# yuw444/fastF

Measured on AMD Instinct MI355X. Metric: BAM records/sec -> deduped UMI matrix; achieved HBM GB/s vs roofline, higher is better.
Workload: dtype u64

## Files before the change

fastf_amd/csrc/umi_engine.hip:

```cpp
#include "umi_kernels.hpp"

#include <algorithm>
#include <cstdarg>
#include <cstdio>
#include <cstdlib>
#include <cstring>
#include <mutex>
#include <new>
#include <stdexcept>
#include <chrono>
#include <string>
#include <thread>
#include <vector>

extern "C" {
#include "fastf_amd.h"
#include "host_io.h"
#include "mt_jump.h"
}

using namespace fastf;

static std::mutex g_err_mu;
static char g_err[512] = "";
// ... 191 lines not shown
    std::vector<uint8_t> h_unonnull;
    u64 total_records = 0, hits_so_far = 0, keys_so_far = 0;
    u64 c_sampled = 0, c_valid = 0;
    bool finished = false; int sorted_in_tmp = 0; u64 n_sorted = 0;
    u32 skip_bits = 0;
    bool fully_sorted = false;
    DevBuf d_cellidx, d_tilecnt, d_tilebase, d_binbase, d_cnt;
    DevBuf d_halfhits;
    DevBuf d_segkeys;
    DevBuf d_segcount, d_segprefix, d_tileseg;
    u32 giant_parity = 0;
    u32 seg_n = 0; u64 seg_stride = 0;
    DevBuf d_rgn_phys, d_rgn_hist, d_rgn_blk;
    u32 rgn_hist_n = 0, rgn_hist_shift = 0;
    bool stream_mode = false, store_regions = false;
    u64 slots_used = 0, slot_cap = 0; u32 rgn_n = 0, rgn_cap = 0;
    DevBuf d_scanblk;
    DevBuf d_rg_feature, d_rg_cell, d_rg_count, d_rg_ukeys, d_spanrows, d_spanbase, d_giant;
    u32 rg_n = 0; bool rg_umi = false;
    bool wide = false, long_umi = false; u32 group_bits = 0;
    u32 sub_bits = 0, row_split = 0;
    bool finish_queued = false;
    DevBuf d_vals, d_vtmp;
    bool timing = false;
    hipEvent_t t_ev[2] = {nullptr, nullptr};
    double t_scatter_ms = 0; u64 t_scatter_n = 0;
    double t_k1_ms = 0; u64 t_k1_n = 0;
    double t_k1b_ms = 0; u64 t_k1b_n = 0;
    double t_k3_ms = 0; u64 t_k3_n = 0;
    double t_count_ms = 0; u64 t_count_n = 0;
// ... 192 lines not shown
        for (u32 w = 0; w < words; ++w) { rank[w] = (unsigned short)acc; acc += (u32)__builtin_popcount(bitmap[w]); }
    }
    if (e->img_genes.ensure(bytes)) return 1;
    if (copy_h2d(e->img_genes.p, img.data(), bytes)) return 1;
    e->lds_genes.image = (const u32*)e->img_genes.p; e->lds_genes.words = words; e->lds_genes.n_perm = (u32)best_n;
    e->lds_genes.family = (u32)best; e->lds_genes.vmin = vmin; e->lds_genes.range = range; e->lds_genes.bytes = (u32)bytes; e->lds_genes.direct = direct ? 1u : 0u;
    {
        const void* fns[] = {(const void*)filter_pack_kernel<true, false>, (const void*)filter_pack_kernel<true, true>,
                             (const void*)filter_pack_stream_kernel<false, false, false>, (const void*)filter_pack_stream_kernel<false, false, true>,
                             (const void*)filter_pack_stream_kernel<false, true, false>, (const void*)filter_pack_stream_kernel<false, true, true>,
                             (const void*)filter_pack_stream_kernel<true, false, false>, (const void*)filter_pack_stream_kernel<true, false, true>,
                             (const void*)filter_pack_stream_kernel<true, true, false>, (const void*)filter_pack_stream_kernel<true, true, true>,
                             (const void*)filter_pack_stream_kernel<false, false, false, true>, (const void*)filter_pack_stream_kernel<false, false, true, true>,
                             (const void*)filter_pack_stream_kernel<false, true, false, true>, (const void*)filter_pack_stream_kernel<false, true, true, true>,
                             (const void*)filter_pack_stream_kernel<true, false, false, true>, (const void*)filter_pack_stream_kernel<true, false, true, true>,
                             (const void*)filter_pack_stream_kernel<true, true, false, true>, (const void*)filter_pack_stream_kernel<true, true, true, true>};
        for (const void* f : fns)
            if (hipFuncSetAttribute(f, hipFuncAttributeMaxDynamicSharedMemorySize, (int)bytes) != hipSuccess) return 0;
    }
    const size_t per_block = bytes + 1024;
    e->genes_blocks_per_cu = (u32)std::max<size_t>(1, std::min<size_t>(3, (160 * 1024) / per_block));
    e->use_lds_genes = true;
    return 0;
}

extern "C" int fastf_engine_create(const fastf_engine_config_t* cfg, fastf_engine_t** out) FASTF_TRY {
    if (!cfg || !out) return set_err("null argument");
    *out = nullptr;
    const char* pf_ = getenv("FASTF_PROFILE");
    const bool lap_on = pf_ && pf_[0] == '2';
    const auto t_0 = std::chrono::steady_clock::now();
    auto lap = [&](const char* what) { if (lap_on) fprintf(stderr, "[engine create] %s at %.1f ms\n", what, std::chrono::duration<double, std::milli>(std::chrono::steady_clock::now() - t_0).count()); };
    int ndev = 0;
    hipError_t he = hipGetDeviceCount(&ndev);
    lap("device count");
    if (he != hipSuccess || ndev == 0)
        return set_err("no HIP device available (%s): the engine has no CPU fallback", hipGetErrorString(he));
// ... 76 lines not shown
        }
        lap("tables built and uploaded");
        if ((rc = e->d_small.ensure(SM_WORDS * sizeof(u64)))) break;
        if (hipHostMalloc((void**)&e->h_small, SM_WORDS * sizeof(u64), hipHostMallocDefault) != hipSuccess) {
            rc = set_err("hipHostMalloc failed"); break;
        }
        if (hipMemset(e->d_small.p, 0, SM_WORDS * sizeof(u64)) != hipSuccess) { rc = set_err("memset failed"); break; }
        lap("counters allocated and cleared");
        if (set_scatter_lds_limit()) {
            rc = set_err("cannot raise dynamic LDS limit to %zu bytes", scatter_smem_bytes()); break;
        }
        lap("kernel attributes (code object loaded)");
        e->batch_cap = cfg->batch_records ? cfg->batch_records : (4ull << 20);
        e->key_cap = cfg->key_capacity;
        e->stream_mode = e->use_lds_genes && !e->wide && e->n_shards == 1 && !getenv("FASTF_NO_STREAM_K1B") && !getenv("FASTF_PUSH_TILE_FORM");
    } while (0);
    if (rc) { fastf_engine_destroy(e); return 1; }
    *out = e;
    return 0;
} FASTF_CATCH_INT

extern "C" void fastf_engine_destroy(fastf_engine_t* e) FASTF_TRY {
    if (!e) return;
    if (e->multi) { multi_destroy(e); delete e; return; }
    (void)hipSetDevice(e->device);
    (void)hipDeviceSynchronize();
    for (int i = 0; i < 2; ++i) {
        fastf_engine::Slot& sl = e->slot[i];
        if (sl.h_stage) (void)hipHostFree(sl.h_stage);
        if (sl.h_draws) (void)hipHostFree(sl.h_draws);
// ... 130 lines not shown
    constexpr u32 CHUNK = 16u * 1024u;
    const u32 n_blk = (T + CHUNK - 1) / CHUNK;
    if (n_blk <= 1 || n_blk > 64 || e->d_scanblk.ensure(2 * 64 * sizeof(u64))) {
        hipLaunchKernelGGL(scan_tiles_kernel<16>, dim3(1), dim3(1024), 0, s, in, out, T, total_out, running, base_out, (u64*)nullptr);
        return;
    }
    u64* const blk = (u64*)e->d_scanblk.p + 64 * slot;
    hipLaunchKernelGGL(scan_tiles_kernel<16>, dim3(n_blk), dim3(1024), 0, s, in, out, T, (u64*)nullptr, (u64*)nullptr, (u64*)nullptr, blk);
    hipLaunchKernelGGL(scan_fix_kernel<16>, dim3(n_blk), dim3(1024), 0, s, out, T, (const u64*)blk, n_blk, total_out, running, base_out);
}

static int launch_probe_cells(fastf_engine* e, const u64* cb, u64 n, u64* d_total_out, hipStream_t s,
                              u64* d_running = nullptr, u64* d_base_out = nullptr, void* blk = nullptr) {
    if (reserve_workspace(e, blk ? 0 : n, 0, n)) return 1;
    const u32 tiles = (u32)((n + K1_TILE - 1) / K1_TILE);
    const CellOut cout = blk ? CellOut{blk, blk_run_bytes(e->cell16)} : CellOut{e->d_cellidx.p, 0u};
    t_begin(e, s);
    if (e->use_lds_cells) {
        const u32 grid = std::min<u32>(e->cells_blocks_per_cu * g_cu_count, (tiles + 1) / 2);
        if (e->cells_blocks_per_cu >= 2)
            hipLaunchKernelGGL(probe_cells_lds_kernel<true>, dim3(grid), dim3(1024), e->lds_cells.bytes, s, cb, n, e->lds_cells,
                               cout, e->cell16, (u32*)e->d_tilecnt.p, (u32*)e->d_halfhits.p, tiles);
        else
            hipLaunchKernelGGL(probe_cells_lds_kernel<false>, dim3(grid), dim3(1024), e->lds_cells.bytes, s, cb, n, e->lds_cells,
                               cout, e->cell16, (u32*)e->d_tilecnt.p, (u32*)e->d_halfhits.p, tiles);
    } else if (e->cell_filter.bits) {
        const u32 grid = std::min<u32>(tiles, 4 * g_cu_count);
        hipLaunchKernelGGL(probe_cells_filtered_kernel, dim3(grid), dim3(K1_THREADS), (e->cell_filter.mask + 1u) / 8u, s, cb, n,
                           e->cells, e->cell_filter, cout, e->cell16, (u32*)e->d_tilecnt.p, (u32*)e->d_halfhits.p, tiles);
    } else {
        hipLaunchKernelGGL(probe_cells_kernel<0>, dim3(tiles), dim3(K1_THREADS), 0, s, cb, n, e->cells,
// ... 13 lines not shown
    if (e->multi) return set_err("fastf_dev_count_hits: device-level calls take a single-device engine");
    HIP_OK(hipSetDevice(e->device));
    hipStream_t s = (hipStream_t)stream;
    if (n == 0) { HIP_OK(hipMemsetAsync(d_hits_out, 0, sizeof(u64), s)); return 0; }
    return launch_probe_cells(e, (const u64*)d_cb_key, n, (u64*)d_hits_out, s);
} FASTF_CATCH_INT

static bool stream_k1b_possible(const fastf_engine* e) {
    return e->use_lds_genes && e->n_shards <= (u32)MAX_SHARDS && !getenv("FASTF_NO_STREAM_K1B");
}

extern "C" int fastf_dev_block_bytes(const fastf_engine_t* e, uint64_t n, uint64_t* bytes) FASTF_TRY {
    if (!e || !bytes) return set_err("null argument");
    *bytes = 0;
    if (e->multi || e->wide || !stream_k1b_possible(e)) return 0;
    *bytes = ((n + BLK_RECS - 1) / BLK_RECS) * (u64)blk_run_bytes(e->cell16);
    return 0;
} FASTF_CATCH_INT

extern "C" int fastf_dev_block_records(fastf_engine_t* e, const uint64_t* d_gx_key, const uint32_t* d_umi, const uint32_t* d_meta,
                                       uint64_t n, void* d_blocked, void* stream) FASTF_TRY {
    if (!e || !d_blocked) return set_err("null argument");
    if (e->multi) return set_err("fastf_dev_block_records: device-level calls take a single-device engine");
    HIP_OK(hipSetDevice(e->device));
    if (n == 0) return 0;
    const u64 units = (n + BLK_RECS - 1) / BLK_RECS;
    hipLaunchKernelGGL(block_records_kernel, dim3((u32)std::min<u64>((units + 3) / 4, 16ull * g_cu_count)), dim3(256), 0, (hipStream_t)stream,
                       (const u64*)d_gx_key, d_umi, d_meta, (u64)n, (unsigned char*)d_blocked, blk_run_bytes(e->cell16));
    HIP_OK(hipGetLastError());
    dbg_sync((hipStream_t)stream, "block_records");
    return 0;
} FASTF_CATCH_INT

extern "C" int fastf_dev_count_hits_blocked(fastf_engine_t* e, const uint64_t* d_cb_key, uint64_t n, void* d_blocked,
                                            uint64_t* d_hits_out, void* stream) FASTF_TRY {
    if (!e || !d_blocked) return set_err("null argument");
    if (e->multi) return set_err("fastf_dev_count_hits_blocked: device-level calls take a single-device engine");
    HIP_OK(hipSetDevice(e->device));
    hipStream_t s = (hipStream_t)stream;
    if (n == 0) { HIP_OK(hipMemsetAsync(d_hits_out, 0, sizeof(u64), s)); return 0; }
    return launch_probe_cells(e, (const u64*)d_cb_key, n, (u64*)d_hits_out, s, nullptr, nullptr, d_blocked);
} FASTF_CATCH_INT

// ... 149 lines not shown
            if (e->d_segkeys.ensure((size_t)n_rgn * region * sizeof(u64))) return 1;
            p.keys = (u64*)e->d_segkeys.p;
        } else if ((u64)n_rgn * region > stride) return set_err("segmented key output needs %llu slots, the buffer has %llu (fastf_dev_probe_capacity)",
                                                                (unsigned long long)((u64)n_rgn * region), (unsigned long long)stride);
        if (app) {
            if (e->rgn_cap < rgn0 + n_rgn) return set_err("internal error: region tables too small");
        } else {
            if (e->rgn_n) return set_err("device-level K1 on an engine that holds pushed chunks: fastf_engine_reset first");
            if (grow_regions(e, n_rgn)) return 1;
        }
        if (e->d_segprefix.ensure(((size_t)n_rgn + 1) * sizeof(u64))) return 1;
        StreamParams sp{(const u32*)e->d_halfhits.p, region, (u64*)e->d_segcount.p + rgn0,
                        stream_shards ? nullptr : (u32*)e->d_rgn_hist.p + (size_t)rgn0 * RADIX, (u64*)e->d_rgn_phys.p + rgn0,
                        app ? app->slot0 : 0ull, e->skip_bits};
        const int variant = (e->genes_blocks_per_cu >= 2 ? 0 : 4) | (e->cell16 ? 2 : 0) | (e->lds_genes.direct ? 1 : 0);
#define FPS(R, C, D) do { if (blk) hipLaunchKernelGGL((filter_pack_stream_kernel<R, C, D, true>), dim3(grid), dim3(R ? K1S_THREADS_ROOMY : K1S_THREADS), e->lds_genes.bytes, s, p, sp); \
                          else hipLaunchKernelGGL((filter_pack_stream_kernel<R, C, D, false>), dim3(grid), dim3(R ? K1S_THREADS_ROOMY : K1S_THREADS), e->lds_genes.bytes, s, p, sp); } while (0)
        switch (variant) {
        case 0: FPS(false, false, false); break; case 1: FPS(false, false, true); break;
        case 2: FPS(false, true, false); break;  case 3: FPS(false, true, true); break;
        case 4: FPS(true, false, false); break;  case 5: FPS(true, false, true); break;
        case 6: FPS(true, true, false); break;   default: FPS(true, true, true); break;
        }
#undef FPS
        if (stream_shards) {
            hipLaunchKernelGGL(shard_partition_kernel, dim3(n_rgn), dim3(SP_THREADS), 0, s, (const u64*)e->d_segkeys.p, (const u64*)e->d_segcount.p,
                               region, e->L.cell_shift, e->n_shards, keys, stride, key_counts, counters + 3);
        } else if (app) {
            hipLaunchKernelGGL(seg_scan_kernel, dim3(1), dim3(1024), 0, s, (const u64*)e->d_segcount.p + rgn0, n_rgn, (u64*)e->d_segprefix.p, key_counts, true);
        } else {
            hipLaunchKernelGGL(seg_scan_kernel, dim3(1), dim3(1024), 0, s, (const u64*)e->d_segcount.p, n_rgn, (u64*)e->d_segprefix.p, key_counts, false);
// ... 333 lines not shown
           "block_records_kernel,tile_count_kernel,row_scan_kernel,scatter_kernel,reduce_windows_kernel,reduce_hashed_kernel,span_scan_kernel,"
           "giant_groups_kernel,rows_gather_kernel";
} FASTF_CATCH_ZERO

static const char* err_bits_text(u64 bits) {
    static thread_local char buf[256];
    snprintf(buf, sizeof buf, "device error bits 0x%llx:%s%s%s%s%s", (unsigned long long)bits,
             (bits & 1) ? " (unknown bit 0);" : "",
             (bits & ERR_DRAWS_SHORT) ? " draw stream shorter than CB hits;" : "",
             (bits & ERR_UMI_TOOLONG) ? " UMI longer than umi_max_bases (raise it: up to 32, with fastf_batch_t.umi_ext from 17 on);" : "",
             (bits & ERR_KEYS_FULL) ? " key store full;" : "",
             (bits & ERR_RUN_TOO_LONG) ? " unsorted run longer than the group-only path handles: sort fully (drop FASTF_SORT_SKIP_LOW);" : "");
    return buf;
}

static size_t stage_bytes(u64 cap) { return (size_t)cap * (8 + 8 + 4 + 4 + 4) + 8192; }


static int slot_alloc(fastf_engine* e, fastf_engine::Slot& sl, bool need_host_stage) {
    if (!sl.h_small) HIP_OK(hipHostMalloc((void**)&sl.h_small, SM_WORDS * sizeof(u64), hipHostMallocDefault));
    if (sl.d_stage.ensure(stage_bytes(e->batch_cap))) return 1;
    if (need_host_stage && !sl.h_stage) HIP_OK(hipHostMalloc(&sl.h_stage, stage_bytes(e->batch_cap), hipHostMallocDefault));
    return 0;
}

static int retire_slot(fastf_engine* e, fastf_engine::Slot& sl) {
    if (!sl.busy) return 0;
    HIP_OK(hipEventSynchronize(sl.ev_done));
    sl.busy = false;
    e->inflight_records -= sl.n;
    const u64* c = sl.h_small + SM_COUNTERS;
    if (!sl.external) e->mt_hits += c[0] - e->hits_so_far;
    e->hits_so_far = c[0];
    e->c_sampled = c[1]; e->c_valid = c[2];
    e->keys_so_far = sl.h_small[SM_KEYCOUNT];
    if (c[3]) return set_err("%s", err_bits_text(c[3]));
// ... 137 lines not shown
        const bool par = n >= (1u << 18);
        if (par) {
            t_gx = std::thread([=] { memcpy(hs + o_gx, s_gx, n * 8); });
            t_um = std::thread([=] { memcpy(hs + o_umi, s_umi, n * 4); memcpy(hs + o_meta, s_meta, n * 4); });
        } else {
            memcpy(hs + o_gx, s_gx, n * 8); memcpy(hs + o_umi, s_umi, n * 4); memcpy(hs + o_meta, s_meta, n * 4);
        }
        memcpy(hs, s_cb, n * 8);
        if (s_ext) { memcpy(hs + o_ext, s_ext, n * 4); s_ext = hs + o_ext; }
        if (par) { t_gx.join(); t_um.join(); }
        s_cb = hs; s_gx = hs + o_gx; s_umi = hs + o_umi; s_meta = hs + o_meta;
    }
    hipStream_t sc = e->s_copy, sk = e->s_compute;
    HIP_OK(hipMemcpyAsync(ds, s_cb, n * 8, hipMemcpyDefault, sc));
    char* const blk = ds + cap * 8;
    if (e->stream_mode) {
        const u32 run = blk_run_bytes(e->cell16);
        const u64 full = n / BLK_RECS, tail = n % BLK_RECS;
        if (full) {
            HIP_OK(hipMemcpy2DAsync(blk + BLK_GX, run, s_gx, BLK_RECS * 8, BLK_RECS * 8, full, hipMemcpyDefault, sc));
            HIP_OK(hipMemcpy2DAsync(blk + BLK_UMI, run, s_umi, BLK_RECS * 4, BLK_RECS * 4, full, hipMemcpyDefault, sc));
            HIP_OK(hipMemcpy2DAsync(blk + BLK_META, run, s_meta, BLK_RECS * 4, BLK_RECS * 4, full, hipMemcpyDefault, sc));
        }
        if (tail) {
            char* const last = blk + full * run;
            HIP_OK(hipMemcpyAsync(last + BLK_GX, (const char*)s_gx + full * BLK_RECS * 8, tail * 8, hipMemcpyDefault, sc));
            HIP_OK(hipMemcpyAsync(last + BLK_UMI, (const char*)s_umi + full * BLK_RECS * 4, tail * 4, hipMemcpyDefault, sc));
            HIP_OK(hipMemcpyAsync(last + BLK_META, (const char*)s_meta + full * BLK_RECS * 4, tail * 4, hipMemcpyDefault, sc));
        }
    } else {
    HIP_OK(hipMemcpyAsync(ds + o_gx, s_gx, n * 8, hipMemcpyDefault, sc));
// ... 514 lines not shown
```

fastf_amd/csrc/umi_kernels.hpp:

```cpp
#pragma once
#if !defined(FASTF_EXPERIMENT)
#  if defined(FASTF_X_ANY)
#    error "FASTF_X_* knobs need -DFASTF_EXPERIMENT (experiment builds only: tools/build_variant.sh)"
#  endif
#endif
#ifndef FASTF_K1_IPT
#define FASTF_K1_IPT 8
#endif
#ifndef FASTF_K1_THREADS
#define FASTF_K1_THREADS 512
#endif
#include <hip/hip_runtime.h>
#include <stdint.h>
#include <type_traits>

namespace fastf {

typedef unsigned long long u64;
typedef unsigned int u32;

constexpr int WAVE = 64;

constexpr u64 ERR_DRAWS_SHORT  = 2;
constexpr u64 ERR_UMI_TOOLONG  = 4;
// ... 290 lines not shown
        k |= (1ULL << (L.umi_bits + L.len_bits)) | ((u64)(umi >> (32 - L.umi_bits)) << L.len_bits) | len;
    }
    return k;
}

__device__ __forceinline__ u64 make_key_flat(const KeyLayout L, u32 cell, u32 feat, u32 umi, u32 meta) {
    const u32 nn = (meta / META_UMI_NONNULL) & 1u, len = (meta & META_LEN_MASK) >> META_LEN_SHIFT;
    const u64 low = ((u64)nn << (L.umi_bits + L.len_bits)) | ((u64)(umi >> (32 - L.umi_bits)) << L.len_bits) | len;
    return ((u64)cell << L.cell_shift) | ((u64)feat << L.feat_shift) | (low & (0ull - (u64)nn));
}
__device__ __forceinline__ bool umi_overflows_flat(const KeyLayout L, u32 umi, u32 meta) {
    const u32 tail = L.umi_bits < 32 ? (1u << (32 - L.umi_bits)) - 1u : 0u;
    const u32 len = (meta & META_LEN_MASK) >> META_LEN_SHIFT;
    return ((meta & META_UMI_TOOLONG) != 0) | (((meta & META_UMI_NONNULL) != 0) & ((len > L.umi_max_bytes) | ((umi & tail) != 0)));
}

__device__ __forceinline__ u64 make_val64(const KeyLayout L, u64 umi, u32 meta) {
    if (!(meta & META_UMI_NONNULL)) return 0;
    const u32 len = (meta & META_LEN_MASK) >> META_LEN_SHIFT;
    return (1ULL << (L.umi_bits + L.len_bits)) | ((umi >> (64 - L.umi_bits)) << L.len_bits) | len;
}
constexpr u32 WIDE_SUB_BITS = 17, WIDE_SUB_VAL_BITS = 51, WIDE_SUB_LEN_BITS = 4;
__device__ __forceinline__ u64 make_val_sub(u64 umi, u32 meta) {
    if (!(meta & META_UMI_NONNULL)) return 0;
    const u32 len = (meta & META_LEN_MASK) >> META_LEN_SHIFT;
    return (1ULL << WIDE_SUB_VAL_BITS) | (((umi << WIDE_SUB_LEN_BITS) | len) & ((1ULL << WIDE_SUB_VAL_BITS) - 1));
}
__device__ __forceinline__ u32 wide_sub_of(u32 umi_first_word, u32 meta) {
    static_assert(WIDE_SUB_VAL_BITS - WIDE_SUB_LEN_BITS + WIDE_SUB_BITS == 64, "the sub-group and the value's bases make up the 64 bits of bases");
    return (meta & META_UMI_NONNULL) ? umi_first_word >> (32 - WIDE_SUB_BITS) : 0u;
// ... 109 lines not shown
    u64 off = 0, total = 0;
    for (u32 i = 0; i < n_blk; ++i) { const u64 v = blk_tot[i]; if (i < blockIdx.x) off += v; total += v; }
    if (blockIdx.x == 0 && threadIdx.x == 0) {
        if (total_out) *total_out = total;
        if (running) { const u64 r = *running; *base_out = r; *running = r + total; }
    }
    if (blockIdx.x == 0 || off == 0) return;
    const u32 t_first = blockIdx.x * PER * 1024u;
    for (u32 k = threadIdx.x; k < PER * 1024u && t_first + k < T; k += 1024) out[t_first + k] += off;
}

constexpr int K1_THREADS = FASTF_K1_THREADS, K1_IPT = FASTF_K1_IPT, K1_TILE = K1_THREADS * K1_IPT, K1_WAVES = K1_THREADS / WAVE;
static_assert(K1_THREADS == 512 && K1_IPT == 8, "K1a layout: 8 waves x 8 items x 64 lanes per tile");

constexpr u32 BLK_RECS = 256, BLK_GX = 0, BLK_UMI = 2048, BLK_META = 3072, BLK_CELL = 4096;
__host__ __device__ __forceinline__ u32 blk_run_bytes(bool c16) { return BLK_CELL + (c16 ? 2u : 4u) * BLK_RECS; }
struct CellOut { void* p; u32 run; };
__device__ __forceinline__ void put_cell(const CellOut o, bool c16, u64 idx, u32 v) {
    unsigned char* at = reinterpret_cast<unsigned char*>(o.p);
    u64 i = idx;
    if (o.run) { at += (idx / BLK_RECS) * o.run + BLK_CELL; i = idx % BLK_RECS; }
    if (c16) reinterpret_cast<unsigned short*>(at)[i] = (unsigned short)v; else reinterpret_cast<u32*>(at)[i] = v;
}
__device__ __forceinline__ u32 get_cell(const void* __restrict__ in, bool c16, u64 idx) {
    return c16 ? (u32)reinterpret_cast<const unsigned short*>(in)[idx] : reinterpret_cast<const u32*>(in)[idx];
}

__device__ __forceinline__ u32 get_cell_once(const void* __restrict__ in, bool c16, u64 idx) {
    return c16 ? (u32)ld_once<FASTF_NT_K1B != 0>(reinterpret_cast<const unsigned short*>(in) + idx)
               : ld_once<FASTF_NT_K1B != 0>(reinterpret_cast<const u32*>(in) + idx);
}

__device__ __forceinline__ u32 shard_of(u32 cell, u32 n_shards) {
    return (u32)((mix64((u64)cell) >> 32) % n_shards);
}

// ... 133 lines not shown
        }
        u32 hits = 0, hits_lo = 0;
#pragma unroll
        for (int j = 0; j < K1_IPT; ++j) {
            const bool fam = (u32)(key[j] >> 49) == c.family && (key[j] & 0xFFFFu) == 0;
            const u32 h = cell_mix((u32)(key[j] >> 16), c.seed);
            const u32 lo = h & lo_mask;
            const u32 e = s_slot[((h >> (32u - S)) + s_disp[lo & c.bucket_mask]) & smask];
            const u32 v = (fam && (e >> S) == lo) ? (e & smask) : 0u;
            cell[j] = v;
            hits += (u32)__popcll(__ballot(v != 0));
            if (j == K1_IPT / 2 - 1) hits_lo = hits;
        }
        if (whole && cell_dst.run) {
            static_assert(K1_IPT * WAVE == 2 * (int)BLK_RECS && PAIRS == 4, "a K1a chunk is two blocked units");
            unsigned char* const u0 = reinterpret_cast<unsigned char*>(cell_out) + (base / BLK_RECS) * cell_dst.run + BLK_CELL;
#pragma unroll
            for (int j = 0; j < PAIRS; ++j) {
                unsigned char* const ub = u0 + (j >> 1) * cell_dst.run;
                const u32 rec = 2u * ((u32)(j & 1) * WAVE + (u32)lane);
                if (c16) *reinterpret_cast<u32*>(ub + 2u * rec) = cell[2 * j] | (cell[2 * j + 1] << 16);
                else *reinterpret_cast<uint2*>(ub + 4u * rec) = make_uint2(cell[2 * j], cell[2 * j + 1]);
            }
        } else if (whole) {
            if (c16) {
#pragma unroll
                for (int j = 0; j < PAIRS; ++j)
                    *reinterpret_cast<u32*>(reinterpret_cast<unsigned short*>(cell_out) + base + 2ull * (j * WAVE + lane)) = cell[2 * j] | (cell[2 * j + 1] << 16);
            } else {
#pragma unroll
                for (int j = 0; j < PAIRS; ++j)
// ... 272 lines not shown
    u64* seg_count;
    u32* rgn_hist;
    u64* rgn_phys;
    u64 slot0;
    u32 hist_shift;
};

__device__ __forceinline__ u32 row16_sum_lane15(u32 x) {
    x += (u32)__builtin_amdgcn_update_dpp(0, (int)x, 0x111, 0xF, 0xF, true);
    x += (u32)__builtin_amdgcn_update_dpp(0, (int)x, 0x112, 0xF, 0xF, true);
    x += (u32)__builtin_amdgcn_update_dpp(0, (int)x, 0x114, 0xF, 0xF, true);
    x += (u32)__builtin_amdgcn_update_dpp(0, (int)x, 0x118, 0xF, 0xF, true);
    return (u32)__builtin_amdgcn_readlane((int)x, 15);
}

template <bool ROOMY, bool C16, bool DIRECT, bool BLOCKED = false>
__global__ __launch_bounds__(ROOMY ? K1S_THREADS_ROOMY : K1S_THREADS, ROOMY ? 4 : 2 * K1S_THREADS / (4 * WAVE)) void filter_pack_stream_kernel(const PackParams p, const StreamParams sp) {
    constexpr int THREADS = ROOMY ? K1S_THREADS_ROOMY : K1S_THREADS, WAVES = THREADS / WAVE;
    __shared__ u64 s_tot[3];
    __shared__ u32 s_cursor[K1S_SUB], s_err;
    __shared__ u32 s_hist[K1S_SUB * K1S_BINS];
    extern __shared__ __attribute__((aligned(16))) unsigned char smem[];
    const int tid = threadIdx.x, lane = lane_id();
    const int w = __builtin_amdgcn_readfirstlane(tid >> 6);
    const u32* s_bitmap = reinterpret_cast<const u32*>(smem);
    const unsigned short* s_rank = reinterpret_cast<const unsigned short*>(smem + (size_t)p.genes.words * 4);
    const unsigned short* s_perm = s_rank + ((p.genes.words + 1u) & ~1u);
    const unsigned short* s_direct = reinterpret_cast<const unsigned short*>(smem);
    {
        const uint4* src = reinterpret_cast<const uint4*>(p.genes.image);
        uint4* dst = reinterpret_cast<uint4*>(smem);
        for (u32 i = tid; i < (p.genes.bytes + 15u) / 16u; i += THREADS) dst[i] = src[i];
    }
    if (tid < 3) s_tot[tid] = 0;
    if (tid < K1S_SUB) s_cursor[tid] = 0;
    if (tid == 0) s_err = 0;
    for (int i = tid; i < K1S_SUB * K1S_BINS; i += THREADS) s_hist[i] = 0;
    __syncthreads();

    constexpr bool NT = FASTF_NT_K1B != 0;
    u64* const region0 = p.keys + (u64)blockIdx.x * K1S_SUB * sp.region_stride;
    const bool hs_hi = sp.hist_shift >= 32u;
    const u64 draw_off = p.draw_base ? *p.draw_base : 0;
    u32 w_hit = 0, w_samp = 0, w_valid = 0, errs = 0;
    const u32 n_units = p.n_tiles * (u32)(K1_TILE / K1S_UNIT), ustep = gridDim.x * (u32)WAVES;
    const u32 n_live = (u32)((p.n + K1S_UNIT - 1) / K1S_UNIT);
    u32 u = blockIdx.x * (u32)WAVES + (u32)w;
    struct UnitRegs { u32 cell[K1S_IPT], umi[K1S_IPT], meta[K1S_IPT], dw, avail, sbit, nvalid; };
    UnitRegs ra, rb;
    u64 gxk[K1S_IPT];
    u64 tb = 0; u32 hha = 0;
    u32 zlane = 0;
    asm volatile("" : "+v"(zlane));
    auto records_of = [&](const u32 uu) { return uu < n_live ? (u32)(p.n - (u64)uu * K1S_UNIT < (u64)K1S_UNIT ? p.n - (u64)uu * K1S_UNIT : (u64)K1S_UNIT) : 0u; };
    auto unit_run = [&](const u32 uu) { return BLOCKED ? p.blk + (u64)uu * blk_run_bytes(C16) : nullptr; };
    auto load_gx = [&](u64 (&g)[K1S_IPT], const u32 uu, const u32 nv) {
        const u64* const gx_u = BLOCKED ? reinterpret_cast<const u64*>(unit_run(uu) + BLK_GX) : p.gx + (u64)uu * K1S_UNIT;
#pragma unroll
        for (int j = 0; j < K1S_IPT; ++j) {
            const u32 o = (u32)j * WAVE + (u32)lane;
            g[j] = ld_once<NT>(gx_u + (BLOCKED || o < nv ? o : nv - 1u));
        }
    };
    auto load_rest = [&](u32 (&c)[K1S_IPT], u32 (&um)[K1S_IPT], u32 (&me)[K1S_IPT], const u32 uu, const u32 nv) {
        const unsigned char* const run = unit_run(uu);
        const u64 base = (u64)uu * K1S_UNIT;
        const u32* const umi_u = BLOCKED ? reinterpret_cast<const u32*>(run + BLK_UMI) : p.umi + base;
        const u32* const meta_u = BLOCKED ? reinterpret_cast<const u32*>(run + BLK_META) : p.meta + base;
        const unsigned short* const c16_u = BLOCKED ? reinterpret_cast<const unsigned short*>(run + BLK_CELL) : reinterpret_cast<const unsigned short*>(p.cell) + base;
        const u32* const c32_u = BLOCKED ? reinterpret_cast<const u32*>(run + BLK_CELL) : reinterpret_cast<const u32*>(p.cell) + base;
#pragma unroll
        for (int j = 0; j < K1S_IPT; ++j) {
            const u32 o = (u32)j * WAVE + (u32)lane, oc = BLOCKED || o < nv ? o : nv - 1u;
            c[j] = C16 ? (u32)ld_once<NT>(c16_u + oc) : ld_once<NT>(c32_u + oc);
            um[j] = ld_once<NT>(umi_u + oc);
            me[j] = ld_once<NT>(meta_u + oc);
        }
    };
    struct Place { u32 avail, sbit; };
    auto place_unit = [&](u32& words, const u32 uu, const u64 tbv, const u32 hhu) {
        const u32 place = uu & 15u;
        const u64 rank0 = uniform64(tbv) + draw_off + row16_sum_lane15((u32)lane < place ? hhu : 0u);
        Place q;
        q.avail = rank0 < p.n_draws ? (u32)(p.n_draws - rank0 < 1024 ? p.n_draws - rank0 : 1024) : 0u;
        q.sbit = (u32)rank0 & 31u;
        const u64 last = p.n_draws ? (p.n_draws - 1) >> 5 : 0, first = rank0 >> 5;
        const u32 room = first < last ? (u32)(last - first < 15 ? last - first : 15) : 0u;
        const u32 off = (u32)lane & 15u;
        const u32 wi = ((u32)(first < last ? first : last) + (off < room ? off : room)) & (u32)(p.draw_mask >> 5);
        words = p.dbits[wi];
        return q;
// ... 3 lines not shown
        tb = p.tile_base[t + zlane];
        hha = sp.half_hits[16ull * t + ((u32)lane & 15u)];
    };
    if (u < n_units) {
        small_inputs(u);
        ra.nvalid = records_of(u);
        const u32 us = ra.nvalid ? u : n_live - 1u, ns = ra.nvalid ? ra.nvalid : records_of(n_live - 1u);
        load_rest(ra.cell, ra.umi, ra.meta, us, ns);
        const Place q = place_unit(ra.dw, u, tb, hha);
        ra.avail = q.avail; ra.sbit = q.sbit;
        small_inputs(u + ustep);
        load_gx(gxk, us, ns);
    }
    auto one_unit = [&](UnitRegs& cur, UnitRegs& nxt, auto sub_c) {
        constexpr int SUB = decltype(sub_c)::value;
        u32 (&cell)[K1S_IPT] = cur.cell; u32 (&umi)[K1S_IPT] = cur.umi; u32 (&meta)[K1S_IPT] = cur.meta;
        const u32 dw = cur.dw, avail = cur.avail, sbit = cur.sbit, nvalid = cur.nvalid;
        const u32 un = u + ustep;
        const u32 nv_n = un < n_units ? records_of(un) : 0u;
        const u32 us = nv_n ? un : n_live - 1u, ns = nv_n ? nv_n : records_of(n_live - 1u);
        const Place qn = place_unit(nxt.dw, un < n_units ? un : u, tb, hha);
        nxt.avail = qn.avail; nxt.sbit = qn.sbit; nxt.nvalid = nv_n;
        load_rest(nxt.cell, nxt.umi, nxt.meta, us, ns);
        small_inputs(un + ustep);
        __builtin_amdgcn_sched_barrier(0);
        if (nvalid < (u32)K1S_UNIT) {
#pragma unroll
            for (int j = 0; j < K1S_IPT; ++j) cell[j] = (u32)j * WAVE + (u32)lane < nvalid ? cell[j] : 0u;
        }
        u32 keep[K1S_IPT];
        {
// ... 3 lines not shown
            w_hit += H;
            u32 pre = 0;
#pragma unroll
            for (int j = 0; j < K1S_IPT; ++j) {
                const u32 rl = pre + rank_below(hm[j]);
                const u32 bpos = sbit + rl;
                keep[j] = ((u32)__builtin_amdgcn_ds_bpermute((int)((bpos >> 5) << 2), (int)dw) >> (bpos & 31u)) & 1u;
                if (H > avail) cell[j] = rl >= avail ? 0u : cell[j];
                pre += (u32)__popcll(hm[j]);
            }
            if (H > avail) errs |= (u32)ERR_DRAWS_SHORT;
        }
        u32 feat[K1S_IPT];
#pragma unroll
        for (int j = 0; j < K1S_IPT; ++j) {
            const u64 k = gxk[j];
            const bool want = (cell[j] != 0) & ((meta[j] & META_XF_OK) != 0) & (k != 0);
            const bool fam = (u32)(k >> 44) == p.genes.family;
            const u64 v = (k & 0xFFFFFFFFFFFull) - p.genes.vmin;
            const bool in = want & fam & (v < p.genes.range);
            const u32 vi = in ? (u32)v : 0u;
            u32 f;
            if (DIRECT) f = s_direct[vi];
            else {
                const u32 wd = s_bitmap[vi >> 5], rk = s_rank[vi >> 5], bit = vi & 31u;
                const u32 pi = ((wd >> bit) & 1u) ? rk + __popc(wd & ((1u << bit) - 1u)) : 0u;
                f = ((wd >> bit) & 1u) ? s_perm[pi] : 0u;
            }
            f = in ? f : 0u;
            if (__ballot(want & !fam)) { if (want & !fam) f = table_probe(p.feats, k); }
            feat[j] = f;
        }
        __builtin_amdgcn_sched_barrier(0);
        load_gx(gxk, us, ns);
        __builtin_amdgcn_sched_barrier(0);
        u64 key[K1S_IPT], em[K1S_IPT];
        u32 n_keys = 0;
#pragma unroll
        for (int j = 0; j < K1S_IPT; ++j) {
            bool alive = (cell[j] != 0) & (keep[j] != 0);
            w_samp += (u32)__popcll(__ballot(alive));
            alive = alive & (feat[j] != 0) & ((meta[j] & META_HAS_UB) != 0);
            if (__ballot(alive & umi_overflows_flat(p.L, umi[j], meta[j]))) errs |= (u32)ERR_UMI_TOOLONG;
            key[j] = make_key_flat(p.L, cell[j], feat[j], umi[j], meta[j]);
            em[j] = __ballot(alive);
            n_keys += (u32)__popcll(em[j]);
        }
        w_valid += n_keys;
        if (n_keys) {
            u32 pos0 = 0;
            if (lane == 0) pos0 = atomicAdd(&s_cursor[SUB], n_keys);
            pos0 = (u32)__builtin_amdgcn_readfirstlane((int)pos0);
            if ((u64)pos0 + n_keys > sp.region_stride) errs |= (u32)ERR_KEYS_FULL;
            else {
                u64* const region = region0 + (u64)SUB * sp.region_stride;
#pragma unroll
                for (int j = 0; j < K1S_IPT; ++j) {
                    if (__builtin_amdgcn_inverse_ballot_w64(em[j])) {
                        region[pos0 + rank_below(em[j])] = key[j];
// ... 23 lines not shown
        if (lane == 0 && e) atomicOr(&s_err, e);
    }
    __syncthreads();
    const int te = w * WAVE + lane;
    if (te < 3 && s_tot[te]) atomicAdd(&p.counters[te], s_tot[te]);
    if (te == 3 && s_err) atomicOr(&p.counters[3], (u64)s_err);
    if (te >= 64 && te < 64 + K1S_SUB) {
        const u32 r = blockIdx.x * K1S_SUB + (u32)(te - 64);
        sp.seg_count[r] = s_cursor[te - 64];
        if (sp.rgn_hist) sp.rgn_phys[r] = sp.slot0 + (u64)r * sp.region_stride;
    }
    if (sp.rgn_hist)
        for (int i = te; i < K1S_SUB * K1S_BINS; i += THREADS) sp.rgn_hist[(u64)blockIdx.x * (K1S_SUB * K1S_BINS) + i] = s_hist[i];
}

__global__ __launch_bounds__(256) void block_records_kernel(const u64* __restrict__ gx, const u32* __restrict__ umi, const u32* __restrict__ meta,
                                                            u64 n, unsigned char* __restrict__ blk, u32 run) {
    const u64 units = (n + BLK_RECS - 1) / BLK_RECS, waves = (u64)gridDim.x * (blockDim.x / WAVE);
    const int lane = lane_id();
    for (u64 u = (u64)blockIdx.x * (blockDim.x / WAVE) + (threadIdx.x >> 6); u < units; u += waves) {
        unsigned char* const r = blk + u * run;
#pragma unroll
        for (int j = 0; j < (int)BLK_RECS / WAVE; ++j) {
            const u32 o = (u32)j * WAVE + (u32)lane;
            const u64 i = u * BLK_RECS + o;
            const bool in = i < n;
            reinterpret_cast<u64*>(r + BLK_GX)[o] = in ? gx[i] : 0;
            reinterpret_cast<u32*>(r + BLK_UMI)[o] = in ? umi[i] : 0;
            reinterpret_cast<u32*>(r + BLK_META)[o] = in ? meta[i] : 0;
        }
    }
}

constexpr int SP_THREADS = 256, SP_IPT = 8, SP_TILE = SP_THREADS * SP_IPT, MAX_SHARDS = 8;
__global__ __launch_bounds__(SP_THREADS) void shard_partition_kernel(const u64* __restrict__ seg_keys, const u64* __restrict__ seg_count,
                                                                     u64 region_stride, u32 cell_shift, u32 n_shards,
                                                                     u64* __restrict__ keys_out, u64 shard_stride,
                                                                     u64* __restrict__ key_counts, u64* __restrict__ err) {
    __shared__ u32 s_cnt[MAX_SHARDS];
    __shared__ u64 s_base[MAX_SHARDS];
    const int tid = threadIdx.x;
    const u64 cnt = seg_count[blockIdx.x];
    const u64* src = seg_keys + (u64)blockIdx.x * region_stride;
    for (u64 i0 = 0; i0 < cnt; i0 += SP_TILE) {
// ... 1080 lines not shown
```

Baseline: 96.55 billion.

## Add narrow blocked record layout packing gene id and UMI/meta into 32-bit words

New measurement: 111.1 billion (median of 6 runs). 1.15x the previous value.

```diff
diff --git a/fastf_amd/csrc/umi_engine.hip b/fastf_amd/csrc/umi_engine.hip
--- a/fastf_amd/csrc/umi_engine.hip
+++ b/fastf_amd/csrc/umi_engine.hip
@@ -229,6 +229,7 @@
     DevBuf d_rgn_phys, d_rgn_hist, d_rgn_blk;
     u32 rgn_hist_n = 0, rgn_hist_shift = 0;
     bool stream_mode = false, store_regions = false;
+    bool narrow = false, genes_one_family = false;
     u64 slots_used = 0, slot_cap = 0; u32 rgn_n = 0, rgn_cap = 0;
     DevBuf d_scanblk;
     DevBuf d_rg_feature, d_rg_cell, d_rg_count, d_rg_ukeys, d_spanrows, d_spanbase, d_giant;
@@ -451,13 +452,18 @@
                              (const void*)filter_pack_stream_kernel<false, false, false, true>, (const void*)filter_pack_stream_kernel<false, false, true, true>,
                              (const void*)filter_pack_stream_kernel<false, true, false, true>, (const void*)filter_pack_stream_kernel<false, true, true, true>,
                              (const void*)filter_pack_stream_kernel<true, false, false, true>, (const void*)filter_pack_stream_kernel<true, false, true, true>,
-                             (const void*)filter_pack_stream_kernel<true, true, false, true>, (const void*)filter_pack_stream_kernel<true, true, true, true>};
+                             (const void*)filter_pack_stream_kernel<true, true, false, true>, (const void*)filter_pack_stream_kernel<true, true, true, true>,
+                             (const void*)filter_pack_stream_kernel<false, false, false, true, true>, (const void*)filter_pack_stream_kernel<false, false, true, true, true>,
+                             (const void*)filter_pack_stream_kernel<false, true, false, true, true>, (const void*)filter_pack_stream_kernel<false, true, true, true, true>,
+                             (const void*)filter_pack_stream_kernel<true, false, false, true, true>, (const void*)filter_pack_stream_kernel<true, false, true, true, true>,
+                             (const void*)filter_pack_stream_kernel<true, true, false, true, true>, (const void*)filter_pack_stream_kernel<true, true, true, true, true>};
         for (const void* f : fns)
             if (hipFuncSetAttribute(f, hipFuncAttributeMaxDynamicSharedMemorySize, (int)bytes) != hipSuccess) return 0;
     }
     const size_t per_block = bytes + 1024;
     e->genes_blocks_per_cu = (u32)std::max<size_t>(1, std::min<size_t>(3, (160 * 1024) / per_block));
     e->use_lds_genes = true;
+    e->genes_one_family = best_n == n;
     return 0;
 }
 
@@ -564,6 +570,11 @@
         e->batch_cap = cfg->batch_records ? cfg->batch_records : (4ull << 20);
         e->key_cap = cfg->key_capacity;
         e->stream_mode = e->use_lds_genes && !e->wide && e->n_shards == 1 && !getenv("FASTF_NO_STREAM_K1B") && !getenv("FASTF_PUSH_TILE_FORM");
+        {
+            const char* bw = getenv("FASTF_BLOCK_WIDE");
+            e->narrow = e->stream_mode && e->genes_one_family && e->lds_genes.vmin + e->lds_genes.range <= 0xFFFFFFFFull &&
+                        e->L.umi_bits <= 24 && !(bw && bw[0] == '1');
+        }
     } while (0);
     if (rc) { fastf_engine_destroy(e); return 1; }
     *out = e;
@@ -724,7 +735,7 @@
                               u64* d_running = nullptr, u64* d_base_out = nullptr, void* blk = nullptr) {
     if (reserve_workspace(e, blk ? 0 : n, 0, n)) return 1;
     const u32 tiles = (u32)((n + K1_TILE - 1) / K1_TILE);
-    const CellOut cout = blk ? CellOut{blk, blk_run_bytes(e->cell16)} : CellOut{e->d_cellidx.p, 0u};
+    const CellOut cout = blk ? CellOut{blk, blk_run_bytes(e->cell16, e->narrow), blk_cell_off(e->narrow)} : CellOut{e->d_cellidx.p, 0u, 0u};
     t_begin(e, s);
     if (e->use_lds_cells) {
         const u32 grid = std::min<u32>(e->cells_blocks_per_cu * g_cu_count, (tiles + 1) / 2);
@@ -768,9 +779,18 @@
     if (!e || !bytes) return set_err("null argument");
     *bytes = 0;
     if (e->multi || e->wide || !stream_k1b_possible(e)) return 0;
-    *bytes = ((n + BLK_RECS - 1) / BLK_RECS) * (u64)blk_run_bytes(e->cell16);
-    return 0;
-} FASTF_CATCH_INT
+    *bytes = ((n + BLK_RECS - 1) / BLK_RECS) * (u64)blk_run_bytes(e->cell16, e->narrow);
+    return 0;
+} FASTF_CATCH_INT
+
+static void launch_block_records(const fastf_engine* e, const u64* gx, const u32* umi, const u32* meta, u64 n, void* blk, hipStream_t s) {
+    const u64 units = (n + BLK_RECS - 1) / BLK_RECS;
+    const dim3 grid((u32)std::min<u64>((units + 3) / 4, 16ull * g_cu_count));
+    if (e->narrow) hipLaunchKernelGGL(block_records_kernel<true>, grid, dim3(256), 0, s, gx, umi, meta, n, (unsigned char*)blk,
+                                      blk_run_bytes(e->cell16, true), e->lds_genes.family, e->L);
+    else hipLaunchKernelGGL(block_records_kernel<false>, grid, dim3(256), 0, s, gx, umi, meta, n, (unsigned char*)blk,
+                            blk_run_bytes(e->cell16, false), 0u, e->L);
+}
 
 extern "C" int fastf_dev_block_records(fastf_engine_t* e, const uint64_t* d_gx_key, const uint32_t* d_umi, const uint32_t* d_meta,
                                        uint64_t n, void* d_blocked, void* stream) FASTF_TRY {
@@ -778,9 +798,7 @@
     if (e->multi) return set_err("fastf_dev_block_records: device-level calls take a single-device engine");
     HIP_OK(hipSetDevice(e->device));
     if (n == 0) return 0;
-    const u64 units = (n + BLK_RECS - 1) / BLK_RECS;
-    hipLaunchKernelGGL(block_records_kernel, dim3((u32)std::min<u64>((units + 3) / 4, 16ull * g_cu_count)), dim3(256), 0, (hipStream_t)stream,
-                       (const u64*)d_gx_key, d_umi, d_meta, (u64)n, (unsigned char*)d_blocked, blk_run_bytes(e->cell16));
+    launch_block_records(e, (const u64*)d_gx_key, d_umi, d_meta, n, d_blocked, (hipStream_t)stream);
     HIP_OK(hipGetLastError());
     dbg_sync((hipStream_t)stream, "block_records");
     return 0;
@@ -960,7 +978,8 @@
                         stream_shards ? nullptr : (u32*)e->d_rgn_hist.p + (size_t)rgn0 * RADIX, (u64*)e->d_rgn_phys.p + rgn0,
                         app ? app->slot0 : 0ull, e->skip_bits};
         const int variant = (e->genes_blocks_per_cu >= 2 ? 0 : 4) | (e->cell16 ? 2 : 0) | (e->lds_genes.direct ? 1 : 0);
-#define FPS(R, C, D) do { if (blk) hipLaunchKernelGGL((filter_pack_stream_kernel<R, C, D, true>), dim3(grid), dim3(R ? K1S_THREADS_ROOMY : K1S_THREADS), e->lds_genes.bytes, s, p, sp); \
+#define FPS(R, C, D) do { if (blk && e->narrow) hipLaunchKernelGGL((filter_pack_stream_kernel<R, C, D, true, true>), dim3(grid), dim3(R ? K1S_THREADS_ROOMY : K1S_THREADS), e->lds_genes.bytes, s, p, sp); \
+                          else if (blk) hipLaunchKernelGGL((filter_pack_stream_kernel<R, C, D, true>), dim3(grid), dim3(R ? K1S_THREADS_ROOMY : K1S_THREADS), e->lds_genes.bytes, s, p, sp); \
                           else hipLaunchKernelGGL((filter_pack_stream_kernel<R, C, D, false>), dim3(grid), dim3(R ? K1S_THREADS_ROOMY : K1S_THREADS), e->lds_genes.bytes, s, p, sp); } while (0)
         switch (variant) {
         case 0: FPS(false, false, false); break; case 1: FPS(false, false, true); break;
@@ -1324,12 +1343,13 @@
     return buf;
 }
 
-static size_t stage_bytes(u64 cap) { return (size_t)cap * (8 + 8 + 4 + 4 + 4) + 8192; }
+static size_t stage_bytes(u64 cap, bool narrow = false) { return (size_t)cap * (8 + 8 + 4 + 4 + 4 + (narrow ? 8 : 0)) + 8192; }
+static size_t narrow_landing(u64 cap) { return (size_t)cap * 20 + 4096; }
 
 
 static int slot_alloc(fastf_engine* e, fastf_engine::Slot& sl, bool need_host_stage) {
     if (!sl.h_small) HIP_OK(hipHostMalloc((void**)&sl.h_small, SM_WORDS * sizeof(u64), hipHostMallocDefault));
-    if (sl.d_stage.ensure(stage_bytes(e->batch_cap))) return 1;
+    if (sl.d_stage.ensure(stage_bytes(e->batch_cap, e->narrow))) return 1;
     if (need_host_stage && !sl.h_stage) HIP_OK(hipHostMalloc(&sl.h_stage, stage_bytes(e->batch_cap), hipHostMallocDefault));
     return 0;
 }
@@ -1497,7 +1517,24 @@
     hipStream_t sc = e->s_copy, sk = e->s_compute;
     HIP_OK(hipMemcpyAsync(ds, s_cb, n * 8, hipMemcpyDefault, sc));
     char* const blk = ds + cap * 8;
-    if (e->stream_mode) {
+    if (e->stream_mode && e->narrow) {
+        const u64* n_gx = (const u64*)s_gx; const u32* n_umi = (const u32*)s_umi; const u32* n_meta = (const u32*)s_meta;
+        bool on_device = false;
+        if (pinned) {
+            hipPointerAttribute_t a; memset(&a, 0, sizeof a);
+            if (hipPointerGetAttributes(&a, s_gx) == hipSuccess) on_device = a.type == hipMemoryTypeDevice;
+            else (void)hipGetLastError();
+        }
+        if (!on_device) {
+            char* const land = ds + narrow_landing(cap);
+            HIP_OK(hipMemcpyAsync(land, s_gx, n * 8, hipMemcpyDefault, sc));
+            HIP_OK(hipMemcpyAsync(land + cap * 8, s_umi, n * 4, hipMemcpyDefault, sc));
+            HIP_OK(hipMemcpyAsync(land + cap * 12, s_meta, n * 4, hipMemcpyDefault, sc));
+            n_gx = (const u64*)land; n_umi = (const u32*)(land + cap * 8); n_meta = (const u32*)(land + cap * 12);
+        }
+        launch_block_records(e, n_gx, n_umi, n_meta, n, blk, sc);
+        HIP_OK(hipGetLastError());
+    } else if (e->stream_mode) {
         const u32 run = blk_run_bytes(e->cell16);
         const u64 full = n / BLK_RECS, tail = n % BLK_RECS;
         if (full) {
diff --git a/fastf_amd/csrc/umi_kernels.hpp b/fastf_amd/csrc/umi_kernels.hpp
--- a/fastf_amd/csrc/umi_kernels.hpp
+++ b/fastf_amd/csrc/umi_kernels.hpp
@@ -328,6 +328,10 @@
     const u32 len = (meta & META_LEN_MASK) >> META_LEN_SHIFT;
     return ((meta & META_UMI_TOOLONG) != 0) | (((meta & META_UMI_NONNULL) != 0) & ((len > L.umi_max_bytes) | ((umi & tail) != 0)));
 }
+__device__ __forceinline__ bool umi_overflows_narrow(const KeyLayout L, u32 um) {
+    const u32 len = (um & META_LEN_MASK) >> META_LEN_SHIFT;
+    return ((um & META_UMI_TOOLONG) != 0) | (((um & META_UMI_NONNULL) != 0) & (len > L.umi_max_bytes));
+}
 
 __device__ __forceinline__ u64 make_val64(const KeyLayout L, u64 umi, u32 meta) {
     if (!(meta & META_UMI_NONNULL)) return 0;
@@ -467,12 +471,14 @@
 static_assert(K1_THREADS == 512 && K1_IPT == 8, "K1a layout: 8 waves x 8 items x 64 lanes per tile");
 
 constexpr u32 BLK_RECS = 256, BLK_GX = 0, BLK_UMI = 2048, BLK_META = 3072, BLK_CELL = 4096;
-__host__ __device__ __forceinline__ u32 blk_run_bytes(bool c16) { return BLK_CELL + (c16 ? 2u : 4u) * BLK_RECS; }
-struct CellOut { void* p; u32 run; };
+constexpr u32 NBLK_GX = 0, NBLK_UM = 1024, NBLK_CELL = 2048;
+__host__ __device__ __forceinline__ u32 blk_cell_off(bool narrow) { return narrow ? NBLK_CELL : BLK_CELL; }
+__host__ __device__ __forceinline__ u32 blk_run_bytes(bool c16, bool narrow = false) { return blk_cell_off(narrow) + (c16 ? 2u : 4u) * BLK_RECS; }
+struct CellOut { void* p; u32 run; u32 off; };
 __device__ __forceinline__ void put_cell(const CellOut o, bool c16, u64 idx, u32 v) {
     unsigned char* at = reinterpret_cast<unsigned char*>(o.p);
     u64 i = idx;
-    if (o.run) { at += (idx / BLK_RECS) * o.run + BLK_CELL; i = idx % BLK_RECS; }
+    if (o.run) { at += (idx / BLK_RECS) * o.run + o.off; i = idx % BLK_RECS; }
     if (c16) reinterpret_cast<unsigned short*>(at)[i] = (unsigned short)v; else reinterpret_cast<u32*>(at)[i] = v;
 }
 __device__ __forceinline__ u32 get_cell(const void* __restrict__ in, bool c16, u64 idx) {
@@ -636,7 +642,7 @@
         }
         if (whole && cell_dst.run) {
             static_assert(K1_IPT * WAVE == 2 * (int)BLK_RECS && PAIRS == 4, "a K1a chunk is two blocked units");
-            unsigned char* const u0 = reinterpret_cast<unsigned char*>(cell_out) + (base / BLK_RECS) * cell_dst.run + BLK_CELL;
+            unsigned char* const u0 = reinterpret_cast<unsigned char*>(cell_out) + (base / BLK_RECS) * cell_dst.run + cell_dst.off;
 #pragma unroll
             for (int j = 0; j < PAIRS; ++j) {
                 unsigned char* const ub = u0 + (j >> 1) * cell_dst.run;
@@ -939,8 +945,9 @@
     return (u32)__builtin_amdgcn_readlane((int)x, 15);
 }
 
-template <bool ROOMY, bool C16, bool DIRECT, bool BLOCKED = false>
+template <bool ROOMY, bool C16, bool DIRECT, bool BLOCKED = false, bool NARROW = false>
 __global__ __launch_bounds__(ROOMY ? K1S_THREADS_ROOMY : K1S_THREADS, ROOMY ? 4 : 2 * K1S_THREADS / (4 * WAVE)) void filter_pack_stream_kernel(const PackParams p, const StreamParams sp) {
+    static_assert(BLOCKED || !NARROW, "the narrow records exist as blocked runs only");
     constexpr int THREADS = ROOMY ? K1S_THREADS_ROOMY : K1S_THREADS, WAVES = THREADS / WAVE;
     __shared__ u64 s_tot[3];
     __shared__ u32 s_cursor[K1S_SUB], s_err;
@@ -971,35 +978,39 @@
     const u32 n_units = p.n_tiles * (u32)(K1_TILE / K1S_UNIT), ustep = gridDim.x * (u32)WAVES;
     const u32 n_live = (u32)((p.n + K1S_UNIT - 1) / K1S_UNIT);
     u32 u = blockIdx.x * (u32)WAVES + (u32)w;
-    struct UnitRegs { u32 cell[K1S_IPT], umi[K1S_IPT], meta[K1S_IPT], dw, avail, sbit, nvalid; };
+    struct UnitRegs { u32 cell[K1S_IPT], umi[K1S_IPT], meta[NARROW ? 1 : K1S_IPT], dw, avail, sbit, nvalid; };
     UnitRegs ra, rb;
-    u64 gxk[K1S_IPT];
+    using GxT = std::conditional_t<NARROW, u32, u64>;
+    GxT gxk[K1S_IPT];
     u64 tb = 0; u32 hha = 0;
     u32 zlane = 0;
     asm volatile("" : "+v"(zlane));
     auto records_of = [&](const u32 uu) { return uu < n_live ? (u32)(p.n - (u64)uu * K1S_UNIT < (u64)K1S_UNIT ? p.n - (u64)uu * K1S_UNIT : (u64)K1S_UNIT) : 0u; };
-    auto unit_run = [&](const u32 uu) { return BLOCKED ? p.blk + (u64)uu * blk_run_bytes(C16) : nullptr; };
-    auto load_gx = [&](u64 (&g)[K1S_IPT], const u32 uu, const u32 nv) {
-        const u64* const gx_u = BLOCKED ? reinterpret_cast<const u64*>(unit_run(uu) + BLK_GX) : p.gx + (u64)uu * K1S_UNIT;
+    auto unit_run = [&](const u32 uu) { return BLOCKED ? p.blk + (u64)uu * blk_run_bytes(C16, NARROW) : nullptr; };
+    auto meta_of = [&](const UnitRegs& r, const int j) -> u32 { if constexpr (NARROW) return r.umi[j]; else return r.meta[j]; };
+    auto load_gx = [&](GxT (&g)[K1S_IPT], const u32 uu, const u32 nv) {
+        const GxT* gx_u;
+        if constexpr (BLOCKED) gx_u = reinterpret_cast<const GxT*>(unit_run(uu) + (NARROW ? NBLK_GX : BLK_GX));
+        else gx_u = p.gx + (u64)uu * K1S_UNIT;
 #pragma unroll
         for (int j = 0; j < K1S_IPT; ++j) {
             const u32 o = (u32)j * WAVE + (u32)lane;
             g[j] = ld_once<NT>(gx_u + (BLOCKED || o < nv ? o : nv - 1u));
         }
     };
-    auto load_rest = [&](u32 (&c)[K1S_IPT], u32 (&um)[K1S_IPT], u32 (&me)[K1S_IPT], const u32 uu, const u32 nv) {
+    auto load_rest = [&](u32 (&c)[K1S_IPT], u32 (&um)[K1S_IPT], u32 (&me)[NARROW ? 1 : K1S_IPT], const u32 uu, const u32 nv) {
         const unsigned char* const run = unit_run(uu);
         const u64 base = (u64)uu * K1S_UNIT;
-        const u32* const umi_u = BLOCKED ? reinterpret_cast<const u32*>(run + BLK_UMI) : p.umi + base;
+        const u32* const umi_u = BLOCKED ? reinterpret_cast<const u32*>(run + (NARROW ? NBLK_UM : BLK_UMI)) : p.umi + base;
         const u32* const meta_u = BLOCKED ? reinterpret_cast<const u32*>(run + BLK_META) : p.meta + base;
-        const unsigned short* const c16_u = BLOCKED ? reinterpret_cast<const unsigned short*>(run + BLK_CELL) : reinterpret_cast<const unsigned short*>(p.cell) + base;
-        const u32* const c32_u = BLOCKED ? reinterpret_cast<const u32*>(run + BLK_CELL) : reinterpret_cast<const u32*>(p.cell) + base;
+        const unsigned short* const c16_u = BLOCKED ? reinterpret_cast<const unsigned short*>(run + blk_cell_off(NARROW)) : reinterpret_cast<const unsigned short*>(p.cell) + base;
+        const u32* const c32_u = BLOCKED ? reinterpret_cast<const u32*>(run + blk_cell_off(NARROW)) : reinterpret_cast<const u32*>(p.cell) + base;
 #pragma unroll
         for (int j = 0; j < K1S_IPT; ++j) {
             const u32 o = (u32)j * WAVE + (u32)lane, oc = BLOCKED || o < nv ? o : nv - 1u;
             c[j] = C16 ? (u32)ld_once<NT>(c16_u + oc) : ld_once<NT>(c32_u + oc);
             um[j] = ld_once<NT>(umi_u + oc);
-            me[j] = ld_once<NT>(meta_u + oc);
+            if constexpr (!NARROW) me[j] = ld_once<NT>(meta_u + oc);
         }
     };
     struct Place { u32 avail, sbit; };
@@ -1033,7 +1044,7 @@
     }
     auto one_unit = [&](UnitRegs& cur, UnitRegs& nxt, auto sub_c) {
         constexpr int SUB = decltype(sub_c)::value;
-        u32 (&cell)[K1S_IPT] = cur.cell; u32 (&umi)[K1S_IPT] = cur.umi; u32 (&meta)[K1S_IPT] = cur.meta;
+        u32 (&cell)[K1S_IPT] = cur.cell; u32 (&umi)[K1S_IPT] = cur.umi;
         const u32 dw = cur.dw, avail = cur.avail, sbit = cur.sbit, nvalid = cur.nvalid;
         const u32 un = u + ustep;
         const u32 nv_n = un < n_units ? records_of(un) : 0u;
@@ -1067,12 +1078,20 @@
         u32 feat[K1S_IPT];
 #pragma unroll
         for (int j = 0; j < K1S_IPT; ++j) {
-            const u64 k = gxk[j];
-            const bool want = (cell[j] != 0) & ((meta[j] & META_XF_OK) != 0) & (k != 0);
-            const bool fam = (u32)(k >> 44) == p.genes.family;
-            const u64 v = (k & 0xFFFFFFFFFFFull) - p.genes.vmin;
-            const bool in = want & fam & (v < p.genes.range);
-            const u32 vi = in ? (u32)v : 0u;
+            const GxT k = gxk[j];
+            const bool want = (cell[j] != 0) & ((meta_of(cur, j) & META_XF_OK) != 0) & (k != 0);
+            bool fam = true, in;
+            u32 vi;
+            if constexpr (NARROW) {
+                const u32 v = (u32)k - 1u - (u32)p.genes.vmin;
+                in = want & (v < (u32)p.genes.range);
+                vi = in ? v : 0u;
+            } else {
+                fam = (u32)(k >> 44) == p.genes.family;
+                const u64 v = (k & 0xFFFFFFFFFFFull) - p.genes.vmin;
+                in = want & fam & (v < p.genes.range);
+                vi = in ? (u32)v : 0u;
+            }
             u32 f;
             if (DIRECT) f = s_direct[vi];
             else {
@@ -1081,7 +1100,9 @@
                 f = ((wd >> bit) & 1u) ? s_perm[pi] : 0u;
             }
             f = in ? f : 0u;
-            if (__ballot(want & !fam)) { if (want & !fam) f = table_probe(p.feats, k); }
+            if constexpr (!NARROW) {
+                if (__ballot(want & !fam)) { if (want & !fam) f = table_probe(p.feats, k); }
+            }
             feat[j] = f;
         }
         __builtin_amdgcn_sched_barrier(0);
@@ -1093,9 +1114,11 @@
         for (int j = 0; j < K1S_IPT; ++j) {
             bool alive = (cell[j] != 0) & (keep[j] != 0);
             w_samp += (u32)__popcll(__ballot(alive));
-            alive = alive & (feat[j] != 0) & ((meta[j] & META_HAS_UB) != 0);
-            if (__ballot(alive & umi_overflows_flat(p.L, umi[j], meta[j]))) errs |= (u32)ERR_UMI_TOOLONG;
-            key[j] = make_key_flat(p.L, cell[j], feat[j], umi[j], meta[j]);
+            const u32 mj = meta_of(cur, j);
+            alive = alive & (feat[j] != 0) & ((mj & META_HAS_UB) != 0);
+            const bool ovf = NARROW ? umi_overflows_narrow(p.L, umi[j]) : umi_overflows_flat(p.L, umi[j], mj);
+            if (__ballot(alive & ovf)) errs |= (u32)ERR_UMI_TOOLONG;
+            key[j] = make_key_flat(p.L, cell[j], feat[j], umi[j], mj);
             em[j] = __ballot(alive);
             n_keys += (u32)__popcll(em[j]);
         }
@@ -1149,8 +1172,9 @@
         for (int i = te; i < K1S_SUB * K1S_BINS; i += THREADS) sp.rgn_hist[(u64)blockIdx.x * (K1S_SUB * K1S_BINS) + i] = s_hist[i];
 }
 
+template <bool NARROW>
 __global__ __launch_bounds__(256) void block_records_kernel(const u64* __restrict__ gx, const u32* __restrict__ umi, const u32* __restrict__ meta,
-                                                            u64 n, unsigned char* __restrict__ blk, u32 run) {
+                                                            u64 n, unsigned char* __restrict__ blk, u32 run, u32 family, const KeyLayout L) {
     const u64 units = (n + BLK_RECS - 1) / BLK_RECS, waves = (u64)gridDim.x * (blockDim.x / WAVE);
     const int lane = lane_id();
     for (u64 u = (u64)blockIdx.x * (blockDim.x / WAVE) + (threadIdx.x >> 6); u < units; u += waves) {
@@ -1160,9 +1184,17 @@
             const u32 o = (u32)j * WAVE + (u32)lane;
             const u64 i = u * BLK_RECS + o;
             const bool in = i < n;
-            reinterpret_cast<u64*>(r + BLK_GX)[o] = in ? gx[i] : 0;
-            reinterpret_cast<u32*>(r + BLK_UMI)[o] = in ? umi[i] : 0;
-            reinterpret_cast<u32*>(r + BLK_META)[o] = in ? meta[i] : 0;
+            if constexpr (NARROW) {
+                const u64 k = in ? gx[i] : 0;
+                const u32 um = in ? umi[i] : 0, me = in ? meta[i] : 0;
+                const u64 v = k & 0xFFFFFFFFFFFull;
+                reinterpret_cast<u32*>(r + NBLK_GX)[o] = ((k != 0) & ((u32)(k >> 44) == family) & (v < 0xFFFFFFFFull)) ? (u32)v + 1u : 0u;
+                reinterpret_cast<u32*>(r + NBLK_UM)[o] = (um & ~0xFFu) | (me & 0xFFu) | (umi_overflows_flat(L, um, me) ? META_UMI_TOOLONG : 0u);
+            } else {
+                reinterpret_cast<u64*>(r + BLK_GX)[o] = in ? gx[i] : 0;
+                reinterpret_cast<u32*>(r + BLK_UMI)[o] = in ? umi[i] : 0;
+                reinterpret_cast<u32*>(r + BLK_META)[o] = in ? meta[i] : 0;
+            }
         }
     }
 }
```
